# alazarteka/Self-Forcing

Hardware: AMD Instinct MI355X
Metric: decoded frames/sec/node, Wan-1.3B 832x480 4-step AR rollout (higher is better)
Workload: dtype bf16

## Files before the change

### self-forcing_amd/csrc/gemm_bf16.hip

```cpp
#include <type_traits>
#include "sf_common.h"
#include "lds_dma.h"
#include "../../include/sf_hip.h"

namespace {

constexpr int BM = 128, BN = 128, BK = 64;
constexpr int GEMM_THREADS = 256;
constexpr int TILE_BYTES = BM * BK * 2;
constexpr int STAGE_BYTES = 2 * TILE_BYTES;
constexpr int GEMM_LDS = 2 * STAGE_BYTES;

struct GemmP {
  const bf16_t* a;
  const bf16_t* w;
  const bf16_t* bias;
  bf16_t* out;
  const bf16_t* resid;
  const bf16_t* gate_mod;
  const bf16_t* gate_e0;
  long gate_group_stride;
  int rows_per_group;
  int M, N, K, lda, ldw, ldo, ldr;
  int tiles_m, tiles_n;
  long a_bs, w_bs, o_bs, r_bs;
  const float* a_scale;
  const float* w_scale;
  int rows_per_seg;
};

typedef int i32x4 __attribute__((ext_vector_type(4)));
typedef int i32x8 __attribute__((ext_vector_type(8)));

__device__ __forceinline__ f32x4 mfma_f8(const bf16x8& w0, const bf16x8& w1, const bf16x8& x0, const bf16x8& x1, const f32x4& acc) {
  const i32x8 wv = __builtin_shufflevector(__builtin_bit_cast(i32x4, w0), __builtin_bit_cast(i32x4, w1), 0, 1, 2, 3, 4, 5, 6, 7);
  const i32x8 xv = __builtin_shufflevector(__builtin_bit_cast(i32x4, x0), __builtin_bit_cast(i32x4, x1), 0, 1, 2, 3, 4, 5, 6, 7);
  return __builtin_amdgcn_mfma_scale_f32_16x16x128_f8f6f4(wv, xv, acc, 0, 0, 0, 127, 0, 127);
}

template <int MT>
__device__ __forceinline__ void fp8_scale_acc(const GemmP& p, f32x4 (&acc)[MT][4], int m_base, int n_base, int lane) {
  f32x4 ws[4];
#pragma unroll
  for (int nt = 0; nt < 4; ++nt) ws[nt] = *reinterpret_cast<const f32x4*>(p.w_scale + min(n_base + nt * 16 + (lane >> 4) * 4, p.N - 4));
#pragma unroll
  for (int mt = 0; mt < MT; ++mt) {
    const float sa = p.a_scale[min(m_base + mt * 16 + (lane & 15), p.M - 1) / p.rows_per_seg];
#pragma unroll
    for (int nt = 0; nt < 4; ++nt)
#pragma unroll
      for (int j = 0; j < 4; ++j) acc[mt][nt][j] = acc[mt][nt][j] * (sa * ws[nt][j]);
  }
}

template <int GROUP_M>
__device__ __forceinline__ void gemm_tile_of(const GemmP& p, int& tm, int& tn) {
  const int nwg = gridDim.x, bid = blockIdx.x;
  const int wg = sf_xcd_remap(bid, nwg);
  const int width = GROUP_M * p.tiles_n;
  const int group = wg / width, first_m = group * GROUP_M;
  const int gsz = min(p.tiles_m - first_m, GROUP_M);
  const int in_group = wg - group * width;
  tm = first_m + in_group % gsz;
  tn = in_group / gsz;
}

template <int EPI, class Ops>
__device__ __forceinline__ bf16x4 epi_math(const f32x4& a4, const Ops& ops) {
  float y[4];
#pragma unroll
  for (int j = 0; j < 4; ++j) y[j] = a4[j];
  if (ops.has_bias()) {
    const bf16x4 b = ops.bias();
#pragma unroll
    for (int j = 0; j < 4; ++j) y[j] += (float)b[j];
  }
  if (EPI == SF_EPI_BIAS_GELU) {
#pragma unroll
    for (int j = 0; j < 4; ++j) y[j] = gelu_tanh_f(y[j]);
  }
  if (EPI == SF_EPI_BIAS_GATE_RESID) {
    const bf16x4 gm = ops.gate_mod();
    const bf16x4 ge = ops.gate_e0();
#pragma unroll
    for (int j = 0; j < 4; ++j) y[j] *= (float)(bf16_t)((float)gm[j] + (float)ge[j]);
  }
  if (EPI == SF_EPI_BIAS_RESID || EPI == SF_EPI_BIAS_GATE_RESID) {
    const bf16x4 rv = ops.resid();
#pragma unroll
    for (int j = 0; j < 4; ++j) y[j] += (float)rv[j];
  }
  bf16x4 o;
#pragma unroll
  for (int j = 0; j < 4; ++j) o[j] = (bf16_t)y[j];
  return o;
}

struct EpiLoads {
  const GemmP& p;
  int m, n;
  const bf16_t* e0row;
  __device__ __forceinline__ bool has_bias() const { return p.bias != nullptr; }
  __device__ __forceinline__ bf16x4 bias() const { return *reinterpret_cast<const bf16x4*>(p.bias + n); }
  __device__ __forceinline__ bf16x4 gate_mod() const { return *reinterpret_cast<const bf16x4*>(p.gate_mod + n); }
  __device__ __forceinline__ bf16x4 gate_e0() const { return *reinterpret_cast<const bf16x4*>(e0row + n); }
  __device__ __forceinline__ bf16x4 resid() const { return *reinterpret_cast<const bf16x4*>(p.resid + (long)m * p.ldr + n); }
};

struct EpiRegs {
  bf16x4 b, gm, ge, rv;
  __device__ __forceinline__ bool has_bias() const { return true; }
  __device__ __forceinline__ bf16x4 bias() const { return b; }
  __device__ __forceinline__ bf16x4 gate_mod() const { return gm; }
  __device__ __forceinline__ bf16x4 gate_e0() const { return ge; }
  __device__ __forceinline__ bf16x4 resid() const { return rv; }
};

template <int EPI, int MT>
__device__ __forceinline__ void gemm_epilogue(const GemmP& p, f32x4 (&acc)[MT][4], int mrow, int ncol) {
#pragma unroll
  for (int mt = 0; mt < MT; ++mt) {
    const int m = mrow + mt * 16;
    if (m >= p.M) continue;
    const bf16_t* e0row = nullptr;
    if (EPI == SF_EPI_BIAS_GATE_RESID) e0row = p.gate_e0 + (long)(m / p.rows_per_group) * p.gate_group_stride;
#pragma unroll
    for (int nt = 0; nt < 4; ++nt) {
      const int n = ncol + nt * 16;
      if (n >= p.N) continue;
      if (EPI == SF_EPI_F32) {
        *reinterpret_cast<f32x4*>(reinterpret_cast<float*>(p.out) + (long)m * p.ldo + n) = acc[mt][nt];
        continue;
      }
      *reinterpret_cast<bf16x4*>(p.out + (long)m * p.ldo + n) = epi_math<EPI>(acc[mt][nt], EpiLoads{p, m, n, e0row});
    }
  }
}

template <int EPI, int MT>
__device__ __forceinline__ void gemm_epilogue_lds(const GemmP& p, f32x4 (&acc)[MT][4], int m_base, int n_base, char* wbuf, int lane) {
  const int r16 = lane & 15, cg = lane >> 4;
  constexpr bool GATE = EPI == SF_EPI_BIAS_GATE_RESID;
  constexpr bool RESID = EPI == SF_EPI_BIAS_RESID || EPI == SF_EPI_BIAS_GATE_RESID;
  const bf16x4 zero4 = {(bf16_t)0.f, (bf16_t)0.f, (bf16_t)0.f, (bf16_t)0.f};
  int ncol[4];
  bf16x4 bias_v[4], gm_v[4];
#pragma unroll
  for (int nt = 0; nt < 4; ++nt) {
    ncol[nt] = min(n_base + nt * 16 + cg * 4, p.N - 4);
    bias_v[nt] = zero4;
    gm_v[nt] = zero4;
  }
  if (p.bias) {
#pragma unroll
    for (int nt = 0; nt < 4; ++nt) bias_v[nt] = *reinterpret_cast<const bf16x4*>(p.bias + ncol[nt]);
  }
  if (GATE) {
#pragma unroll
    for (int nt = 0; nt < 4; ++nt) gm_v[nt] = *reinterpret_cast<const bf16x4*>(p.gate_mod + ncol[nt]);
  }
  constexpr int MB = 4;
#pragma unroll
  for (int m0 = 0; m0 < MT; m0 += MB) {
    bf16x4 rv[MB][4], ge[MB][4];
#pragma unroll
    for (int i = 0; i < MB; ++i) {
      if (m0 + i >= MT) break;
      const int m = min(m_base + (m0 + i) * 16 + r16, p.M - 1);
      const bf16_t* e0row = GATE ? p.gate_e0 + (long)(m / p.rows_per_group) * p.gate_group_stride : nullptr;
#pragma unroll
      for (int nt = 0; nt < 4; ++nt) {
        rv[i][nt] = RESID ? *reinterpret_cast<const bf16x4*>(p.resid + (long)m * p.ldr + ncol[nt]) : zero4;
        ge[i][nt] = GATE ? *reinterpret_cast<const bf16x4*>(e0row + ncol[nt]) : zero4;
      }
    }
#pragma unroll
    for (int i = 0; i < MB; ++i) {
      if (m0 + i >= MT) break;
      const int row = (m0 + i) * 16 + r16;
#pragma unroll
      for (int nt = 0; nt < 4; ++nt) {
        const int col = nt * 16 + cg * 4;
        const bf16x4 o = epi_math<EPI>(acc[m0 + i][nt], EpiRegs{bias_v[nt], gm_v[nt], ge[i][nt], rv[i][nt]});
        const int chunk = (col >> 3) ^ (row & 7);
        *reinterpret_cast<bf16x4*>(wbuf + row * 128 + (chunk << 4) + (col & 4) * 2) = o;
      }
    }
  }
  __builtin_amdgcn_s_waitcnt(0xc07f);
  const int rr = lane >> 3, ch = lane & 7;
#pragma unroll
  for (int i = 0; i < 2 * MT; ++i) {
    const int row = i * 8 + rr;
    const int m = m_base + row, n = n_base + ch * 8;
    const bf16x8 v = *reinterpret_cast<const bf16x8*>(wbuf + row * 128 + ((ch ^ (row & 7)) << 4));
    if (m < p.M && n < p.N) *reinterpret_cast<bf16x8*>(p.out + (long)m * p.ldo + n) = v;
  }
}

template <int EPI, bool F8>
__global__ __launch_bounds__(GEMM_THREADS, 2) void gemm_bf16_kernel(GemmP p) {
  extern __shared__ __attribute__((aligned(16))) char smem[];
  const int tid = threadIdx.x;
  const int lane = tid & 63;
  const int wave = __builtin_amdgcn_readfirstlane(tid >> 6);

  if (blockIdx.y) {
    const long bz = blockIdx.y;
    p.a += bz * p.a_bs; p.w += bz * p.w_bs;
    if (EPI == SF_EPI_F32) p.out = reinterpret_cast<bf16_t*>(reinterpret_cast<float*>(p.out) + bz * p.o_bs); else p.out += bz * p.o_bs;
    if (p.resid) p.resid += bz * p.r_bs;
  }
  int tm, tn;
  gemm_tile_of<8>(p, tm, tn);
  const int m0 = tm * BM, n0 = tn * BN;

  const bf16_t* a_src[4];
  const bf16_t* w_src[4];
#pragma unroll
  for (int i = 0; i < 4; ++i) {
    const int r = (wave * 4 + i) * 8 + (lane >> 3);
    const int c = (lane & 7) ^ ((r >> 1) & 7);
    const int am = min(m0 + r, p.M - 1);
    const int wn = min(n0 + r, p.N - 1);
    a_src[i] = p.a + (long)am * p.lda + c * 8;
    w_src[i] = p.w + (long)wn * p.ldw + c * 8;
  }
  auto stage = [&](int buf, int kt) {
    char* base = smem + buf * STAGE_BYTES + wave * 4096;
    const int k0 = kt * BK;
#pragma unroll
    for (int i = 0; i < 4; ++i) glds16(a_src[i] + k0, base + i * 1024);
#pragma unroll
    for (int i = 0; i < 4; ++i) glds16(w_src[i] + k0, base + TILE_BYTES + i * 1024);
  };

  const int wr = wave >> 1, wc = wave & 1;
  const int i16 = lane & 15, kq = lane >> 4;
  const int swz = (i16 >> 1) & 7;
  const int x_row_off = (wr * 64 + i16) * 128;
  const int w_row_off = TILE_BYTES + (wc * 64 + i16) * 128;
  const int coff0 = ((0 + kq) ^ swz) << 4;
  const int coff1 = ((4 + kq) ^ swz) << 4;

  f32x4 acc[4][4];
#pragma unroll
  for (int i = 0; i < 4; ++i)
#pragma unroll
    for (int j = 0; j < 4; ++j) acc[i][j] = f32x4{0.f, 0.f, 0.f, 0.f};

  const int nk = p.K / BK;
  stage(0, 0);
  __builtin_amdgcn_s_waitcnt(0);
  __syncthreads();

  for (int kt = 0; kt < nk; ++kt) {
    const int cur = kt & 1;
    const char* buf = smem + cur * STAGE_BYTES;
    const int kn = min(kt + 1, nk - 1) * BK;
    char* sbase = smem + (cur ^ 1) * STAGE_BYTES + wave * 4096;
    bf16x8 xf0[4], wf0[4], xf1[4], wf1[4];
    if constexpr (F8) {
#pragma unroll
      for (int t = 0; t < 4; ++t) {
        xf0[t] = *reinterpret_cast<const bf16x8*>(buf + x_row_off + t * 2048 + coff0);
        wf0[t] = *reinterpret_cast<const bf16x8*>(buf + w_row_off + t * 2048 + coff0);
        xf1[t] = *reinterpret_cast<const bf16x8*>(buf + x_row_off + t * 2048 + coff1);
        wf1[t] = *reinterpret_cast<const bf16x8*>(buf + w_row_off + t * 2048 + coff1);
      }
      __builtin_amdgcn_sched_barrier(0);
#pragma unroll
      for (int i = 0; i < 8; ++i) {
        const int mt = i >> 1, nt0 = (i & 1) * 2;
        acc[mt][nt0] = mfma_f8(wf0[nt0], wf1[nt0], xf0[mt], xf1[mt], acc[mt][nt0]);
        acc[mt][nt0 + 1] = mfma_f8(wf0[nt0 + 1], wf1[nt0 + 1], xf0[mt], xf1[mt], acc[mt][nt0 + 1]);
        if (i < 4) glds16(a_src[i] + kn, sbase + i * 1024);
        else glds16(w_src[i - 4] + kn, sbase + TILE_BYTES + (i - 4) * 1024);
        __builtin_amdgcn_sched_barrier(0);
      }
      __syncthreads();
      continue;
    }
#pragma unroll
    for (int t = 0; t < 4; ++t) {
      xf0[t] = *reinterpret_cast<const bf16x8*>(buf + x_row_off + t * 2048 + coff0);
      wf0[t] = *reinterpret_cast<const bf16x8*>(buf + w_row_off + t * 2048 + coff0);
    }
    __builtin_amdgcn_sched_barrier(0);
#pragma unroll
    for (int i = 0; i < 8; ++i) {
      const int mt = i >> 1, nt0 = (i & 1) * 2;
      acc[mt][nt0] = __builtin_amdgcn_mfma_f32_16x16x32_bf16(wf0[nt0], xf0[mt], acc[mt][nt0], 0, 0, 0);
      acc[mt][nt0 + 1] = __builtin_amdgcn_mfma_f32_16x16x32_bf16(wf0[nt0 + 1], xf0[mt], acc[mt][nt0 + 1], 0, 0, 0);
      if (i < 4) {
        xf1[i] = *reinterpret_cast<const bf16x8*>(buf + x_row_off + i * 2048 + coff1);
        glds16(a_src[i] + kn, sbase + i * 1024);
      } else {
        wf1[i - 4] = *reinterpret_cast<const bf16x8*>(buf + w_row_off + (i - 4) * 2048 + coff1);
        glds16(w_src[i - 4] + kn, sbase + TILE_BYTES + (i - 4) * 1024);
      }
      __builtin_amdgcn_sched_barrier(0);
    }
#pragma unroll
    for (int mt = 0; mt < 4; ++mt)
#pragma unroll
      for (int nt = 0; nt < 4; ++nt)
        acc[mt][nt] = __builtin_amdgcn_mfma_f32_16x16x32_bf16(wf1[nt], xf1[mt], acc[mt][nt], 0, 0, 0);
    __builtin_amdgcn_sched_barrier(0);
    __syncthreads();
  }

  if constexpr (F8) fp8_scale_acc<4>(p, acc, m0 + wr * 64, n0 + wc * 64, lane);
  const int mrow = m0 + wr * 64 + (lane & 15);
  const int ncol = n0 + wc * 64 + (lane >> 4) * 4;
  if (EPI != SF_EPI_F32 && (p.N & 7) == 0 && (p.ldo & 7) == 0)
    gemm_epilogue_lds<EPI, 4>(p, acc, m0 + wr * 64, n0 + wc * 64, smem + wave * 8192, lane);
  else
    gemm_epilogue<EPI, 4>(p, acc, mrow, ncol);
}


constexpr int PP_THREADS = 512;

__device__ __forceinline__ void pp_end_load_segment() {
  __builtin_amdgcn_s_waitcnt(0xc07f);
  __builtin_amdgcn_sched_barrier(0);
  __builtin_amdgcn_s_barrier();
  __builtin_amdgcn_sched_barrier(0);
}

template <bool F8, int R0, int NQ, int MT, int NA>
__device__ __forceinline__ void pp_cluster(f32x4 (&acc)[MT][4], const bf16x8 (&af)[NA][2], const bf16x8 (&bfr)[4][2], int c0) {
  __builtin_amdgcn_s_setprio(1);
  if constexpr (F8) {
#pragma unroll
    for (int mt = 0; mt < NQ; ++mt)
#pragma unroll
      for (int nt = 0; nt < 2; ++nt)
        acc[R0 + mt][c0 + nt] = mfma_f8(bfr[c0 + nt][0], bfr[c0 + nt][1], af[mt][0], af[mt][1], acc[R0 + mt][c0 + nt]);
  } else {
#pragma unroll
    for (int ks = 0; ks < 2; ++ks)
#pragma unroll
      for (int mt = 0; mt < NQ; ++mt)
#pragma unroll
        for (int nt = 0; nt < 2; ++nt)
          acc[R0 + mt][c0 + nt] = __builtin_amdgcn_mfma_f32_16x16x32_bf16(bfr[c0 + nt][ks], af[mt][ks], acc[R0 + mt][c0 + nt], 0, 0, 0);
  }
  __builtin_amdgcn_s_setprio(0);
  __builtin_amdgcn_sched_barrier(0);
  __builtin_amdgcn_s_barrier();
  __builtin_amdgcn_sched_barrier(0);
}

template <int MT>
struct PPCfg {
  static constexpr int BM = 32 * MT;
  static constexpr int A_BYTES = BM * 128;
  static constexpr int B_BYTES = 256 * 128;
  static constexpr int STAGE = A_BYTES + B_BYTES;
  static constexpr int LDS = 2 * STAGE;
  static constexpr int PA = (2 * MT + 7) / 8;
};

template <int EPI, int MT, bool F8>
__global__ __launch_bounds__(PP_THREADS) void gemm_pp_kernel(GemmP p) {
  using Cfg = PPCfg<MT>;
  constexpr int BMp = Cfg::BM, PA = Cfg::PA;
  constexpr int HQA = (MT + 1) / 2, HQB = MT / 2;
  extern __shared__ __attribute__((aligned(16))) char smem[];
  const int tid = threadIdx.x;
  const int lane = tid & 63;
  const int wave = __builtin_amdgcn_readfirstlane(tid >> 6);
  const int grp = wave >> 2, wc = wave & 3;

  int tm, tn;
  gemm_tile_of<(MT >= 6 ? 4 : 8)>(p, tm, tn);
  const int m0 = tm * BMp, n0 = tn * 256;

  const bf16_t* a_src[2][PA];
  const bf16_t* w_src[2][2];
#pragma unroll
  for (int h = 0; h < 2; ++h) {
#pragma unroll
    for (int i = 0; i < PA; ++i) {
      const int r = h * (BMp / 2) + (wave + 8 * i) * 8 + (lane >> 3);
      const int c = (lane & 7) ^ ((r >> 1) & 7);
      a_src[h][i] = p.a + (long)min(m0 + r, p.M - 1) * p.lda + c * 8;
    }
#pragma unroll
    for (int i = 0; i < 2; ++i) {
      const int r = h * 128 + (wave + 8 * i) * 8 + (lane >> 3);
      const int c = (lane & 7) ^ ((r >> 1) & 7);
      w_src[h][i] = p.w + (long)min(n0 + r, p.N - 1) * p.ldw + c * 8;
    }
  }
  auto dma_a = [&](int h, int kt) {
    char* base = smem + (kt & 1) * Cfg::STAGE + h * (Cfg::A_BYTES / 2) + wave * 1024;
#pragma unroll
    for (int i = 0; i < PA; ++i)
      if (wave + 8 * i < 2 * MT) glds16(a_src[h][i] + kt * BK, base + i * 8192);
  };
  auto dma_b = [&](int h, int kt) {
    char* base = smem + (kt & 1) * Cfg::STAGE + Cfg::A_BYTES + h * (Cfg::B_BYTES / 2) + wave * 1024;
#pragma unroll
    for (int i = 0; i < 2; ++i) glds16(w_src[h][i] + kt * BK, base + i * 8192);
  };

  const int i16 = lane & 15, kq = lane >> 4;
  const int swz = (i16 >> 1) & 7;
  const int x_row_off = (grp * (BMp / 2) + i16) * 128;
  const int w_row_off = Cfg::A_BYTES + (wc * 64 + i16) * 128;
  const int coff[2] = {((0 + kq) ^ swz) << 4, ((4 + kq) ^ swz) << 4};

  f32x4 acc[MT][4];
#pragma unroll
  for (int i = 0; i < MT; ++i)
#pragma unroll
    for (int j = 0; j < 4; ++j) acc[i][j] = f32x4{0.f, 0.f, 0.f, 0.f};
  bf16x8 af[HQA][2], bfr[4][2];

#ifdef SF_STAMP
  unsigned long long* stamp = (EPI == SF_EPI_BIAS && p.gate_e0) ? reinterpret_cast<unsigned long long*>(const_cast<bf16_t*>(p.gate_e0)) + ((long)blockIdx.x * 2 + grp) * 8 : nullptr;
  if (stamp && (tid & 255) == 0) { stamp[0] = __builtin_amdgcn_s_memtime(); stamp[4] = __builtin_amdgcn_s_memrealtime(); }
#endif
  const int nk = p.K / BK;
  dma_a(0, 0); dma_a(1, 0); dma_b(0, 0); dma_b(1, 0);
  if (nk > 1) { dma_b(0, 1); dma_b(1, 1); asm volatile("s_waitcnt vmcnt(4)" ::: "memory"); }
  else asm volatile("s_waitcnt vmcnt(0)" ::: "memory");
  __builtin_amdgcn_s_barrier();
#ifdef SF_STAMP
  if (stamp && (tid & 255) == 0) stamp[1] = __builtin_amdgcn_s_memtime();
#endif
  if (grp == 1) __builtin_amdgcn_s_barrier();

  auto cluster = [&](auto qc, int c0) {
    constexpr int q = decltype(qc)::value;
    pp_cluster<F8, q * HQA, q == 0 ? HQA : HQB>(acc, af, bfr, c0);
  };
  auto read_a = [&](const char* buf, auto qc) {
    constexpr int q = decltype(qc)::value, NQ = q == 0 ? HQA : HQB;
#pragma unroll
    for (int mt = 0; mt < NQ; ++mt)
#pragma unroll
      for (int ks = 0; ks < 2; ++ks)
        af[mt][ks] = *reinterpret_cast<const bf16x8*>(buf + x_row_off + (q * HQA + mt) * 2048 + coff[ks]);
  };
  auto read_b = [&](const char* buf, int c0) {
#pragma unroll
    for (int nt = 0; nt < 2; ++nt)
#pragma unroll
      for (int ks = 0; ks < 2; ++ks)
        bfr[c0 + nt][ks] = *reinterpret_cast<const bf16x8*>(buf + w_row_off + (c0 + nt) * 2048 + coff[ks]);
  };

  constexpr std::integral_constant<int, 0> Q0{};
  constexpr std::integral_constant<int, 1> Q1{};
  for (int kt = 0; kt < nk; ++kt) {
    const char* buf = smem + (kt & 1) * Cfg::STAGE;
    const bool more1 = kt + 1 < nk, more2 = kt + 2 < nk;
    read_a(buf, Q0);
    read_b(buf, 0);
    if (more1) dma_a(0, kt + 1);
    pp_end_load_segment();
    cluster(Q0, 0);
    read_b(buf, 2);
    if (more1) dma_a(1, kt + 1);
    pp_end_load_segment();
    cluster(Q0, 2);
    read_a(buf, Q1);
    if (more2) dma_b(0, kt + 2);
    pp_end_load_segment();
    cluster(Q1, 2);
    if (more2) {
      dma_b(1, kt + 2);
      asm volatile("s_waitcnt vmcnt(4)" ::: "memory");
    } else {
      asm volatile("s_waitcnt vmcnt(0)" ::: "memory");
    }
    pp_end_load_segment();
    cluster(Q1, 0);
  }
  if (grp == 0) __builtin_amdgcn_s_barrier();
#ifdef SF_STAMP
  if (stamp && (tid & 255) == 0) stamp[2] = __builtin_amdgcn_s_memtime();
#endif

  const int m_base = m0 + grp * (BMp / 2), n_base = n0 + wc * 64;
  if constexpr (F8) fp8_scale_acc<MT>(p, acc, m_base, n_base, lane);
  if ((p.N & 7) == 0 && (p.ldo & 7) == 0)
    gemm_epilogue_lds<EPI, MT>(p, acc, m_base, n_base, smem + wave * (MT * 2048), lane);
  else
    gemm_epilogue<EPI, MT>(p, acc, m_base + (lane & 15), n_base + (lane >> 4) * 4);
#ifdef SF_STAMP
  asm volatile("s_waitcnt vmcnt(0)" ::: "memory");
  if (stamp && (tid & 255) == 0) { stamp[3] = __builtin_amdgcn_s_memtime(); stamp[5] = __builtin_amdgcn_s_memrealtime(); }
#endif
}

constexpr int PP2_A = 128 * 128, PP2_B = 256 * 128;
constexpr int PP2_LDS = 3 * (PP2_A + PP2_B);

template <int EPI, bool F8>
__global__ __launch_bounds__(PP_THREADS) void gemm_pp2_kernel(GemmP p) {
  extern __shared__ __attribute__((aligned(16))) char smem[];
  const int tid = threadIdx.x;
  const int lane = tid & 63;
  const int wave = __builtin_amdgcn_readfirstlane(tid >> 6);
  const int grp = wave >> 2, wc = wave & 3;

  int tm, tn;
  gemm_tile_of<8>(p, tm, tn);
  const int m0 = tm * 128, n0 = tn * 256;

  const bf16_t* a_src[2];
  const bf16_t* w_src[4];
#pragma unroll
  for (int i = 0; i < 2; ++i) {
    const int r = (wave + 8 * i) * 8 + (lane >> 3);
    a_src[i] = p.a + (long)min(m0 + r, p.M - 1) * p.lda + ((lane & 7) ^ ((r >> 1) & 7)) * 8;
  }
#pragma unroll
  for (int i = 0; i < 4; ++i) {
    const int r = (wave + 8 * i) * 8 + (lane >> 3);
    w_src[i] = p.w + (long)min(n0 + r, p.N - 1) * p.ldw + ((lane & 7) ^ ((r >> 1) & 7)) * 8;
  }
  auto dma_a = [&](int slot, int kt) {
    char* base = smem + slot * PP2_A + wave * 1024;
#pragma unroll
    for (int i = 0; i < 2; ++i) glds16(a_src[i] + kt * BK, base + i * 8192);
  };
  auto dma_b = [&](int slot, int kt) {
    char* base = smem + 3 * PP2_A + slot * PP2_B + wave * 1024;
#pragma unroll
    for (int i = 0; i < 4; ++i) glds16(w_src[i] + kt * BK, base + i * 8192);
  };

  const int i16 = lane & 15, kq = lane >> 4;
  const int swz = (i16 >> 1) & 7;
  const int x_row_off = (grp * 64 + i16) * 128;
  const int w_row_off = 3 * PP2_A + (wc * 64 + i16) * 128;
  const int coff[2] = {((0 + kq) ^ swz) << 4, ((4 + kq) ^ swz) << 4};

  f32x4 acc[4][4];
#pragma unroll
  for (int i = 0; i < 4; ++i)
#pragma unroll
    for (int j = 0; j < 4; ++j) acc[i][j] = f32x4{0.f, 0.f, 0.f, 0.f};
  bf16x8 af[4][2], bfr[4][2];

  const int nk = p.K / BK;
  dma_a(0, 0); dma_b(0, 0);
  if (nk > 1) { dma_a(1, 1); dma_b(1, 1); asm volatile("s_waitcnt vmcnt(6)" ::: "memory"); }
  else asm volatile("s_waitcnt vmcnt(0)" ::: "memory");
  __builtin_amdgcn_s_barrier();
  if (grp == 1) __builtin_amdgcn_s_barrier();

  auto cluster = [&](int c0) { pp_cluster<F8, 0, 4>(acc, af, bfr, c0); };

  int slot = 0;
  for (int kt = 0; kt < nk; ++kt) {
    const char* abuf = smem + slot * PP2_A;
    const char* bbuf = smem + slot * PP2_B;
    const int nslot = slot == 0 ? 2 : slot - 1;
    const bool more2 = kt + 2 < nk;
#pragma unroll
    for (int mt = 0; mt < 4; ++mt)
#pragma unroll
      for (int ks = 0; ks < 2; ++ks) af[mt][ks] = *reinterpret_cast<const bf16x8*>(abuf + x_row_off + mt * 2048 + coff[ks]);
#pragma unroll
    for (int nt = 0; nt < 2; ++nt)
#pragma unroll
      for (int ks = 0; ks < 2; ++ks) bfr[nt][ks] = *reinterpret_cast<const bf16x8*>(bbuf + w_row_off + nt * 2048 + coff[ks]);
    if (more2) dma_a(nslot, kt + 2);
    pp_end_load_segment();
    cluster(0);
#pragma unroll
    for (int nt = 2; nt < 4; ++nt)
#pragma unroll
      for (int ks = 0; ks < 2; ++ks) bfr[nt][ks] = *reinterpret_cast<const bf16x8*>(bbuf + w_row_off + nt * 2048 + coff[ks]);
    if (more2) {
      dma_b(nslot, kt + 2);
      asm volatile("s_waitcnt vmcnt(6)" ::: "memory");
    } else {
      asm volatile("s_waitcnt vmcnt(0)" ::: "memory");
    }
    pp_end_load_segment();
    cluster(2);
    slot = slot == 2 ? 0 : slot + 1;
  }
  if (grp == 0) __builtin_amdgcn_s_barrier();

  const int m_base = m0 + grp * 64, n_base = n0 + wc * 64;
  if constexpr (F8) fp8_scale_acc<4>(p, acc, m_base, n_base, lane);
  if ((p.N & 7) == 0 && (p.ldo & 7) == 0)
    gemm_epilogue_lds<EPI, 4>(p, acc, m_base, n_base, smem + wave * 8192, lane);
  else
    gemm_epilogue<EPI, 4>(p, acc, m_base + (lane & 15), n_base + (lane >> 4) * 4);
}

template <class F>
int with_epilogue(int epilogue, const char* name, F&& f) {
  switch (epilogue) {
    case SF_EPI_BIAS: return f(std::integral_constant<int, SF_EPI_BIAS>{});
    case SF_EPI_BIAS_GELU: return f(std::integral_constant<int, SF_EPI_BIAS_GELU>{});
    case SF_EPI_BIAS_RESID: return f(std::integral_constant<int, SF_EPI_BIAS_RESID>{});
    case SF_EPI_BIAS_GATE_RESID: return f(std::integral_constant<int, SF_EPI_BIAS_GATE_RESID>{});
    default: SF_CHECK(false, "%s: unknown epilogue %d", name, epilogue);
  }
}

template <int MT, bool F8>
int launch_pp(GemmP& p, int epilogue, const char* name, hipStream_t s) {
  using Cfg = PPCfg<MT>;
  p.tiles_m = (p.M + Cfg::BM - 1) / Cfg::BM;
  p.tiles_n = (p.N + 255) / 256;
  return with_epilogue(epilogue, name, [&](auto epi) {
    return sf_launch<&gemm_pp_kernel<decltype(epi)::value, MT, F8>, Cfg::LDS>(name, dim3(p.tiles_m * p.tiles_n), dim3(PP_THREADS), Cfg::LDS, s, p);
  });
}

template <bool F8>
int launch_pp2(GemmP& p, int epilogue, const char* name, hipStream_t s) {
  p.tiles_m = (p.M + 127) / 128;
  p.tiles_n = (p.N + 255) / 256;
  return with_epilogue(epilogue, name, [&](auto epi) {
    return sf_launch<&gemm_pp2_kernel<decltype(epi)::value, F8>, PP2_LDS>(name, dim3(p.tiles_m * p.tiles_n), dim3(PP_THREADS), PP2_LDS, s, p);
  });
}

struct PPStructure {
  int st, rows;
  double rel;
  int (*launch)(GemmP&, int, const char*, hipStream_t);
};
template <bool F8>
constexpr PPStructure PP_STRUCTURES[] = {{SF_GEMM_PP256, 256, 1.00, launch_pp<8, F8>},
                                         {SF_GEMM_PP224, 224, 1.02, launch_pp<7, F8>},
                                         {SF_GEMM_PP192, 192, 1.05, launch_pp<6, F8>},
                                         {SF_GEMM_PP128, 128, 1.14, launch_pp2<F8>}};

int check_args(const sf_gemm_args* a, const char* name, int bk) {
  SF_CHECK(a != nullptr, "%s: null args", name);
  SF_CHECK(a->M > 0 && a->N > 0 && a->K > 0, "%s: empty problem M=%d N=%d K=%d", name, a->M, a->N, a->K);
  SF_CHECK(a->K % bk == 0, "%s: K=%d must be a multiple of %d", name, a->K, bk);
  SF_CHECK(a->N % 4 == 0, "%s: N=%d must be a multiple of 4", name, a->N);
  SF_CHECK(a->lda % (bk / 8) == 0 && a->ldw % (bk / 8) == 0 && a->ldo % 4 == 0, "%s: lda/ldw must be multiples of %d, ldo of 4", name, bk / 8);
  SF_CHECK(a->lda >= a->K && a->ldw >= a->K && a->ldo >= a->N, "%s: leading dimension too small", name);
  SF_CHECK(a->a && a->w && a->out, "%s: null tensor", name);
  SF_CHECK(((uintptr_t)a->a % 16 == 0) && ((uintptr_t)a->w % 16 == 0) && ((uintptr_t)a->out % 8 == 0), "%s: misaligned tensor", name);
  if (a->epilogue == SF_EPI_BIAS_RESID || a->epilogue == SF_EPI_BIAS_GATE_RESID) {
    SF_CHECK(a->resid != nullptr && a->ldr >= a->N && a->ldr % 4 == 0, "%s: residual epilogue needs resid/ldr", name);
  }
  if (a->epilogue == SF_EPI_BIAS_GATE_RESID) {
    SF_CHECK(a->gate_mod && a->gate_e0 && a->rows_per_group > 0, "%s: gate epilogue needs gate_mod/gate_e0/rows_per_group", name);
  }
  SF_CHECK(a->structure >= SF_GEMM_AUTO && a->structure <= SF_GEMM_PP192, "%s: unknown structure %d", name, a->structure);
  return 0;
}

template <bool F8>
int run_gemm(const sf_gemm_args* a, GemmP& p, const char* name, hipStream_t s) {
  int st = a->structure;
  const int nk = p.K / BK;
  const bool pp_ok = a->batch <= 1 && a->epilogue != SF_EPI_F32 && nk >= 2;
  if (st == SF_GEMM_AUTO) {
    st = SF_GEMM_T128;
    if (pp_ok && a->M >= 1024 && a->N >= 1024 && a->K >= 512) {
      const long tn = (a->N + 255) / 256;
      double best = 1e30;
      for (const auto& c : PP_STRUCTURES<F8>) {
        const long tiles = (long)((a->M + c.rows - 1) / c.rows) * tn;
        const double cost = (double)((tiles + 255) / 256) * (c.rows / 256.0 * c.rel + 0.04);
        if (cost < best - 1e-9) { best = cost; st = c.st; }
      }
    }
  }
  if (pp_ok)
    for (const auto& c : PP_STRUCTURES<F8>)
      if (c.st == st) return c.launch(p, a->epilogue, name, s);
  const int batch = a->batch > 1 ? a->batch : 1;
  p.a_bs = a->a_bstride; p.w_bs = a->w_bstride; p.o_bs = a->o_bstride; p.r_bs = a->r_bstride;
  SF_CHECK(batch == 1 || (a->a_bstride % 8 == 0 && a->w_bstride % 8 == 0 && a->o_bstride % 4 == 0 && a->r_bstride % 4 == 0),
           "%s: batch strides must keep 16-byte (operands) / 8-byte (output) alignment", name);
  const dim3 grid(p.tiles_m * p.tiles_n, batch), block(GEMM_THREADS);
  if (a->epilogue != SF_EPI_F32)
    return with_epilogue(a->epilogue, name, [&](auto epi) {
      return sf_launch<&gemm_bf16_kernel<decltype(epi)::value, F8>>(name, grid, block, GEMM_LDS, s, p);
    });
  if constexpr (F8) {
    SF_CHECK(false, "%s: the raw fp32 epilogue is bf16-only", name);
  } else {
    SF_CHECK((uintptr_t)a->out % 16 == 0, "%s: fp32 output must be 16-byte aligned", name);
    return sf_launch<&gemm_bf16_kernel<SF_EPI_F32, false>>(name, grid, block, GEMM_LDS, s, p);
  }
}

void fill_params(const sf_gemm_args* a, GemmP& p, int unit) {
  p.a = (const bf16_t*)a->a; p.w = (const bf16_t*)a->w; p.bias = (const bf16_t*)a->bias;
  p.out = (bf16_t*)a->out; p.resid = (const bf16_t*)a->resid;
  p.gate_mod = (const bf16_t*)a->gate_mod; p.gate_e0 = (const bf16_t*)a->gate_e0;
  p.gate_group_stride = a->gate_group_stride; p.rows_per_group = a->rows_per_group;
  p.M = a->M; p.N = a->N; p.K = a->K / unit; p.lda = a->lda / unit; p.ldw = a->ldw / unit; p.ldo = a->ldo; p.ldr = a->ldr;
  p.tiles_n = (a->N + BN - 1) / BN;
  p.tiles_m = (a->M + BM - 1) / BM;
  p.a_scale = nullptr; p.w_scale = nullptr; p.rows_per_seg = 1;
}

}

extern "C" int sf_gemm_bf16(const sf_gemm_args* a, void* stream) {
  if (const int rc = check_args(a, "sf_gemm_bf16", BK)) return rc;
  GemmP p;
  fill_params(a, p, 1);
  return run_gemm<false>(a, p, "sf_gemm_bf16", (hipStream_t)stream);
}

extern "C" int sf_gemm_fp8(const sf_gemm_args* a, const float* a_scale, int rows_per_segment, const float* w_scale, void* stream) {
  if (const int rc = check_args(a, "sf_gemm_fp8", 2 * BK)) return rc;
  SF_CHECK(a->batch <= 1, "sf_gemm_fp8: batched products are bf16-only");
  SF_CHECK(a_scale && w_scale && rows_per_segment > 0, "sf_gemm_fp8: needs a_scale, w_scale and rows_per_segment > 0");
  SF_CHECK((uintptr_t)w_scale % 16 == 0, "sf_gemm_fp8: w_scale must be 16-byte aligned");
  GemmP p;
  fill_params(a, p, 2);
  p.a_scale = a_scale; p.w_scale = w_scale; p.rows_per_seg = rows_per_segment;
  return run_gemm<true>(a, p, "sf_gemm_fp8", (hipStream_t)stream);
}
```

Before: 94.64.

## Stage residual tile via LDS DMA and precompute gate per row group in GEMM epilogue

The LDS epilogue now loads the residual tile with coalesced 16-byte direct-to-LDS DMA into the per-wave write buffer and reads it back with the swizzled layout, replacing strided bf16x4 global loads. When a tile falls within one row group, the gate (gate_mod + e0) is computed once per column instead of per row. An empty asm barrier is added after FP8 scaling to pin the accumulator. The aim is to cut global-memory latency and redundant loads in the fused epilogue. It also adds an alignment check on the residual pointer and stride that falls back to the plain epilogue, plus a slower path for tiles that cross group boundaries.

```diff
diff --git a/self-forcing_amd/csrc/gemm_bf16.hip b/self-forcing_amd/csrc/gemm_bf16.hip
--- a/self-forcing_amd/csrc/gemm_bf16.hip
+++ b/self-forcing_amd/csrc/gemm_bf16.hip
@@ -50,6 +50,8 @@
     for (int nt = 0; nt < 4; ++nt)
 #pragma unroll
       for (int j = 0; j < 4; ++j) acc[mt][nt][j] = acc[mt][nt][j] * (sa * ws[nt][j]);
+#pragma unroll
+    for (int nt = 0; nt < 4; ++nt) asm volatile("" : "+v"(acc[mt][nt]));
   }
 }
 
@@ -65,6 +67,13 @@
   tn = in_group / gsz;
 }
 
+__device__ __forceinline__ bf16x4 epi_gate(const bf16x4& gm, const bf16x4& ge) {
+  bf16x4 g;
+#pragma unroll
+  for (int j = 0; j < 4; ++j) g[j] = (bf16_t)((float)gm[j] + (float)ge[j]);
+  return g;
+}
+
 template <int EPI, class Ops>
 __device__ __forceinline__ bf16x4 epi_math(const f32x4& a4, const Ops& ops) {
   float y[4];
@@ -80,10 +89,9 @@
     for (int j = 0; j < 4; ++j) y[j] = gelu_tanh_f(y[j]);
   }
   if (EPI == SF_EPI_BIAS_GATE_RESID) {
-    const bf16x4 gm = ops.gate_mod();
-    const bf16x4 ge = ops.gate_e0();
-#pragma unroll
-    for (int j = 0; j < 4; ++j) y[j] *= (float)(bf16_t)((float)gm[j] + (float)ge[j]);
+    const bf16x4 gt = ops.gate();
+#pragma unroll
+    for (int j = 0; j < 4; ++j) y[j] *= (float)gt[j];
   }
   if (EPI == SF_EPI_BIAS_RESID || EPI == SF_EPI_BIAS_GATE_RESID) {
     const bf16x4 rv = ops.resid();
@@ -102,17 +110,17 @@
   const bf16_t* e0row;
   __device__ __forceinline__ bool has_bias() const { return p.bias != nullptr; }
   __device__ __forceinline__ bf16x4 bias() const { return *reinterpret_cast<const bf16x4*>(p.bias + n); }
-  __device__ __forceinline__ bf16x4 gate_mod() const { return *reinterpret_cast<const bf16x4*>(p.gate_mod + n); }
-  __device__ __forceinline__ bf16x4 gate_e0() const { return *reinterpret_cast<const bf16x4*>(e0row + n); }
+  __device__ __forceinline__ bf16x4 gate() const {
+    return epi_gate(*reinterpret_cast<const bf16x4*>(p.gate_mod + n), *reinterpret_cast<const bf16x4*>(e0row + n));
+  }
   __device__ __forceinline__ bf16x4 resid() const { return *reinterpret_cast<const bf16x4*>(p.resid + (long)m * p.ldr + n); }
 };
 
 struct EpiRegs {
-  bf16x4 b, gm, ge, rv;
+  bf16x4 b, g, rv;
   __device__ __forceinline__ bool has_bias() const { return true; }
   __device__ __forceinline__ bf16x4 bias() const { return b; }
-  __device__ __forceinline__ bf16x4 gate_mod() const { return gm; }
-  __device__ __forceinline__ bf16x4 gate_e0() const { return ge; }
+  __device__ __forceinline__ bf16x4 gate() const { return g; }
   __device__ __forceinline__ bf16x4 resid() const { return rv; }
 };
 
@@ -137,19 +145,27 @@
   }
 }
 
+template <int EPI>
+__device__ __forceinline__ bool epi_lds_ok(const GemmP& p) {
+  constexpr bool RESID = EPI == SF_EPI_BIAS_RESID || EPI == SF_EPI_BIAS_GATE_RESID;
+  if (EPI == SF_EPI_F32 || (p.N & 7) != 0 || (p.ldo & 7) != 0) return false;
+  return !RESID || ((p.ldr & 7) == 0 && (reinterpret_cast<uintptr_t>(p.resid) & 15) == 0);
+}
+
 template <int EPI, int MT>
 __device__ __forceinline__ void gemm_epilogue_lds(const GemmP& p, f32x4 (&acc)[MT][4], int m_base, int n_base, char* wbuf, int lane) {
   const int r16 = lane & 15, cg = lane >> 4;
+  const int rr = lane >> 3, ch = lane & 7;
   constexpr bool GATE = EPI == SF_EPI_BIAS_GATE_RESID;
   constexpr bool RESID = EPI == SF_EPI_BIAS_RESID || EPI == SF_EPI_BIAS_GATE_RESID;
   const bf16x4 zero4 = {(bf16_t)0.f, (bf16_t)0.f, (bf16_t)0.f, (bf16_t)0.f};
   int ncol[4];
-  bf16x4 bias_v[4], gm_v[4];
+  bf16x4 bias_v[4], gate_v[4];
 #pragma unroll
   for (int nt = 0; nt < 4; ++nt) {
     ncol[nt] = min(n_base + nt * 16 + cg * 4, p.N - 4);
     bias_v[nt] = zero4;
-    gm_v[nt] = zero4;
+    gate_v[nt] = zero4;
   }
   if (p.bias) {
 #pragma unroll
@@ -157,38 +173,66 @@
   }
   if (GATE) {
 #pragma unroll
-    for (int nt = 0; nt < 4; ++nt) gm_v[nt] = *reinterpret_cast<const bf16x4*>(p.gate_mod + ncol[nt]);
-  }
-  constexpr int MB = 4;
-#pragma unroll
-  for (int m0 = 0; m0 < MT; m0 += MB) {
-    bf16x4 rv[MB][4], ge[MB][4];
-#pragma unroll
-    for (int i = 0; i < MB; ++i) {
-      if (m0 + i >= MT) break;
-      const int m = min(m_base + (m0 + i) * 16 + r16, p.M - 1);
-      const bf16_t* e0row = GATE ? p.gate_e0 + (long)(m / p.rows_per_group) * p.gate_group_stride : nullptr;
-#pragma unroll
-      for (int nt = 0; nt < 4; ++nt) {
-        rv[i][nt] = RESID ? *reinterpret_cast<const bf16x4*>(p.resid + (long)m * p.ldr + ncol[nt]) : zero4;
-        ge[i][nt] = GATE ? *reinterpret_cast<const bf16x4*>(e0row + ncol[nt]) : zero4;
+    for (int nt = 0; nt < 4; ++nt) gate_v[nt] = *reinterpret_cast<const bf16x4*>(p.gate_mod + ncol[nt]);
+  }
+  if (RESID) {
+    const bf16_t* src = p.resid + min(n_base + (ch ^ rr) * 8, p.N - 8);
+#pragma unroll
+    for (int i = 0; i < 2 * MT; ++i) glds16(src + (long)min(m_base + i * 8 + rr, p.M - 1) * p.ldr, wbuf + i * 1024);
+    __builtin_amdgcn_sched_barrier(0);
+  }
+  bool one_group = false;
+  if (GATE) {
+    const int first = min(m_base, p.M - 1), last = min(m_base + 16 * MT - 1, p.M - 1);
+    const int group = first / p.rows_per_group;
+    one_group = last - group * p.rows_per_group < p.rows_per_group;
+    if (one_group) {
+      const bf16_t* e0row = p.gate_e0 + (long)group * p.gate_group_stride;
+#pragma unroll
+      for (int nt = 0; nt < 4; ++nt) gate_v[nt] = epi_gate(gate_v[nt], *reinterpret_cast<const bf16x4*>(e0row + ncol[nt]));
+    }
+  }
+  if (RESID) {
+    asm volatile("s_waitcnt vmcnt(0)" ::: "memory");
+    __builtin_amdgcn_s_waitcnt(0xc07f);
+  }
+  auto row_blocks = [&](auto one) {
+    constexpr bool ONE = decltype(one)::value;
+    constexpr int MB = ONE ? 4 : 2;
+#pragma unroll
+    for (int m0 = 0; m0 < MT; m0 += MB) {
+      bf16x4 rv[MB][4], ge[MB][4];
+#pragma unroll
+      for (int i = 0; i < MB; ++i) {
+        if (m0 + i >= MT) break;
+        const int row = (m0 + i) * 16 + r16;
+        const int m = min(m_base + row, p.M - 1);
+        const bf16_t* e0row = GATE && !ONE ? p.gate_e0 + (long)(m / p.rows_per_group) * p.gate_group_stride : nullptr;
+#pragma unroll
+        for (int nt = 0; nt < 4; ++nt) {
+          const int col = nt * 16 + cg * 4;
+          rv[i][nt] = RESID ? *reinterpret_cast<const bf16x4*>(wbuf + row * 128 + (((col >> 3) ^ (row & 7)) << 4) + (col & 4) * 2) : zero4;
+          ge[i][nt] = GATE && !ONE ? *reinterpret_cast<const bf16x4*>(e0row + ncol[nt]) : zero4;
+        }
       }
-    }
-#pragma unroll
-    for (int i = 0; i < MB; ++i) {
-      if (m0 + i >= MT) break;
-      const int row = (m0 + i) * 16 + r16;
-#pragma unroll
-      for (int nt = 0; nt < 4; ++nt) {
-        const int col = nt * 16 + cg * 4;
-        const bf16x4 o = epi_math<EPI>(acc[m0 + i][nt], EpiRegs{bias_v[nt], gm_v[nt], ge[i][nt], rv[i][nt]});
-        const int chunk = (col >> 3) ^ (row & 7);
-        *reinterpret_cast<bf16x4*>(wbuf + row * 128 + (chunk << 4) + (col & 4) * 2) = o;
+#pragma unroll
+      for (int i = 0; i < MB; ++i) {
+        if (m0 + i >= MT) break;
+        const int row = (m0 + i) * 16 + r16;
+#pragma unroll
+        for (int nt = 0; nt < 4; ++nt) {
+          const int col = nt * 16 + cg * 4;
+          const bf16x4 gt = GATE && !ONE ? epi_gate(gate_v[nt], ge[i][nt]) : gate_v[nt];
+          const bf16x4 o = epi_math<EPI>(acc[m0 + i][nt], EpiRegs{bias_v[nt], gt, rv[i][nt]});
+          const int chunk = (col >> 3) ^ (row & 7);
+          *reinterpret_cast<bf16x4*>(wbuf + row * 128 + (chunk << 4) + (col & 4) * 2) = o;
+        }
       }
     }
-  }
+  };
+  if (__builtin_expect(!GATE || one_group, 1)) row_blocks(std::true_type{});
+  else row_blocks(std::false_type{});
   __builtin_amdgcn_s_waitcnt(0xc07f);
-  const int rr = lane >> 3, ch = lane & 7;
 #pragma unroll
   for (int i = 0; i < 2 * MT; ++i) {
     const int row = i * 8 + rr;
@@ -313,7 +357,7 @@
   if constexpr (F8) fp8_scale_acc<4>(p, acc, m0 + wr * 64, n0 + wc * 64, lane);
   const int mrow = m0 + wr * 64 + (lane & 15);
   const int ncol = n0 + wc * 64 + (lane >> 4) * 4;
-  if (EPI != SF_EPI_F32 && (p.N & 7) == 0 && (p.ldo & 7) == 0)
+  if (epi_lds_ok<EPI>(p))
     gemm_epilogue_lds<EPI, 4>(p, acc, m0 + wr * 64, n0 + wc * 64, smem + wave * 8192, lane);
   else
     gemm_epilogue<EPI, 4>(p, acc, mrow, ncol);
@@ -488,7 +532,7 @@
 
   const int m_base = m0 + grp * (BMp / 2), n_base = n0 + wc * 64;
   if constexpr (F8) fp8_scale_acc<MT>(p, acc, m_base, n_base, lane);
-  if ((p.N & 7) == 0 && (p.ldo & 7) == 0)
+  if (epi_lds_ok<EPI>(p))
     gemm_epilogue_lds<EPI, MT>(p, acc, m_base, n_base, smem + wave * (MT * 2048), lane);
   else
     gemm_epilogue<EPI, MT>(p, acc, m_base + (lane & 15), n_base + (lane >> 4) * 4);
@@ -593,7 +637,7 @@
 
   const int m_base = m0 + grp * 64, n_base = n0 + wc * 64;
   if constexpr (F8) fp8_scale_acc<4>(p, acc, m_base, n_base, lane);
-  if ((p.N & 7) == 0 && (p.ldo & 7) == 0)
+  if (epi_lds_ok<EPI>(p))
     gemm_epilogue_lds<EPI, 4>(p, acc, m_base, n_base, smem + wave * 8192, lane);
   else
     gemm_epilogue<EPI, 4>(p, acc, m_base + (lane & 15), n_base + (lane >> 4) * 4);
```

New measurement: 95.22, median of 6. Within noise of the previous version (+0.6%).
